# lenskit/csr

Measured on AMD Instinct MI355X. Metric: spmv_gflops, higher is better.
Workload: dtype f64

## Files before the change

### csr_amd/csrc/spmv.hip

```cpp
#include "spmv_plan.h"

#include <algorithm>
#include <ctime>

namespace csrk {
template <bool R32>
__device__ __forceinline__ double spmv_prod(double a, double x)
{
    const double t = a * x;
    return R32 ? (double)(float)t : t;
}

void free_spmv_plan(SpmvPlan *p) { delete p; }

void spmv_plan_bytes_by_part(const SpmvPlan *p, int64_t out[5])
{
    for (int i = 0; i < 5; i++) out[i] = 0;
    auto add = [&](int part, std::initializer_list<const DevBuf *> bufs) {
        for (const DevBuf *b : bufs) out[part] += (int64_t)b->bytes;
    };
    for (const AccPanel *ap : p->acc) add(0, {&ap->row_list, &ap->vals, &ap->idx, &ap->tile_row0, &ap->segs, &ap->wg_seg, &ap->partial, &ap->z});
    const Panel &t = p->tier1;
    add(1, {&t.row_list, &t.rp, &t.ci, &t.vs, &t.tile, &t.group, &t.carry_row, &t.carry_val, &t.y, &t.crp, &t.cidx});
    const LightStream *l = &p->ls;
    add(2, {&l->vals, &l->idx, &l->rowids, &l->tile_base, &l->carry_row, &l->carry_val});
    add(3, {&l->xg, &l->a_col, &l->a_dst, &l->blk_start, &l->round_start, &l->round_tile0, &l->wg_round0, &p->hot_slot, &p->hot_cols, &p->xh});
    add(4, {&p->tile_row, &p->carry_row, &p->carry_val, &p->rp_light, &p->cut_pos, &p->cut_cum, &p->tile_cut, &p->heavy_row, &p->seg_off,
            &p->seg_row, &p->seg_part, &p->xwide});
}

int64_t spmv_plan_bytes(const SpmvPlan *p)
{
    int64_t part[5];
    spmv_plan_bytes_by_part(p, part);
    return part[0] + part[1] + part[2] + part[3] + part[4];
}
// ... 217 lines not shown
            }
        }
    }
}

template <class XT>
__global__ void hot_pack_kernel(const XT *__restrict__ x, const int32_t *__restrict__ hot_cols, int32_t n_hot,
                                double *__restrict__ xh)
{
    const int i = blockIdx.x * blockDim.x + threadIdx.x;
    if (i < n_hot) xh[i] = (double)x[hot_cols[i]];
}

struct PanelRider {
    int64_t first;
    const double *partial;
    double *z;
    int32_t H, n_wg;
};

template <class PP, int PT, bool R32 = false, class XT = double>
__global__ __launch_bounds__(PT) void spmv_panel_kernel(
    const PP *__restrict__ prp, const int32_t *__restrict__ pci, const double *__restrict__ pvs,
    const XT *__restrict__ x, int32_t ncols, double *__restrict__ yp, const PanelTile *__restrict__ tiles,
    const PanelGroup *__restrict__ groups, int64_t n_prows, int32_t *__restrict__ carry_row,
    double *__restrict__ carry_val, int64_t pnnz, int32_t cb, PanelRider rider)
{
    constexpr uint32_t POS_MASK = (1u << PANEL_POS_BITS) - 1;
    __shared__ double s_buf[MERGE_ITEMS + 1];
    __shared__ int32_t s_long[MERGE_MAXLONG];
    __shared__ int32_t s_nlong;
    __shared__ double s_wpart[PT / WAVE];

    constexpr int PPAIRS = MERGE_ITEMS / PT / 2;
    const int tid = threadIdx.x;
    const int lane = tid & (WAVE - 1), wv = tid / WAVE;
    if ((int64_t)blockIdx.x >= rider.first) {
        constexpr int G = PT / WAVE;
        const int h = (int)((int64_t)blockIdx.x - rider.first) * WAVE + lane;
        const int per = (rider.n_wg + G - 1) / G;
        const int w0 = wv * per, w1 = w0 + per < rider.n_wg ? w0 + per : rider.n_wg;
        double acc = 0.0;
        if (h < rider.H) {
#pragma unroll 8
            for (int w = w0; w < w1; w++) acc += rider.partial[(int64_t)w * rider.H + h];
        }
        s_buf[wv * WAVE + lane] = acc;
        __syncthreads();
        if (wv == 0 && h < rider.H) {
            double tot = s_buf[lane];
            for (int u = 1; u < G; u++) tot += s_buf[u * WAVE + lane];
            rider.z[h] = tot;
        }
        return;
    }
    const PanelGroup grp = groups[blockIdx.x];
    if (grp.nt == 0) return;
    constexpr int RPT = MERGE_ITEMS / PT;
    int32_t c0[PPAIRS], c1[PPAIRS], rv[RPT];
    double p0[PPAIRS], p1[PPAIRS];
    PanelTile pt = tiles[grp.t0];

#define PANEL_LOAD_TILE(T)                                                                            \
    {                                                                                                 \
        const int64_t j0_ = (T).j0;                                                                   \
        const int nn_ = (T).nn, nr_ = (T).i1 - (T).i0;                                                \
        _Pragma("unroll") for (int u = 0; u < PPAIRS; u++)                                       \
// ... 92 lines not shown
            acc = wave_sum(acc);
            if (lane == 0) {
                if (r < nr) {
                    yp[i0 + r] = acc;
                } else {
                    *(pt.cslot >= 0 ? yp + pt.cslot : carry_val + t) = acc;
                }
            }
        }
        pt = nx;
    }
#undef PANEL_LOAD_TILE
}

template <int CB, int PT, bool R32 = false, class SV = double, class XT = double>
__global__ __launch_bounds__(PT) void spmv_acc_kernel(const SV *__restrict__ pvals, const uint16_t *__restrict__ pidx,
                                                     const int32_t *__restrict__ tile_row0,
                                                     const XT *__restrict__ x, int32_t ncols,
                                                     const AccSeg *__restrict__ segs, const int32_t *__restrict__ wg_seg,
                                                     int32_t H, double *__restrict__ partial, int32_t fx_g)
{
    extern __shared__ __align__(16) unsigned char acc_smem[];
    double *s_x = (double *)acc_smem;
    double *s_acc = s_x + CB + 2;
    const int Hpad = (H + 1) & ~1;
    double *s_hval = s_acc + Hpad;
    int32_t *s_hrow = (int32_t *)(s_hval + ACC_SEG_TILES);
    constexpr int NW = PT / WAVE;
    const int tid = threadIdx.x, lane = tid & (WAVE - 1), wv = tid / WAVE;

    for (int h = tid; h < Hpad; h += PT) s_acc[h] = 0.0;
    if (tid < 2) s_x[CB + tid] = 0.0;
    const unsigned long long below = lane ? (~0ull >> (WAVE - lane)) : 0ull;
    const unsigned long long upto = below | (1ull << lane);

    int cur_blk = -1;
    const int sb = wg_seg[blockIdx.x], se = wg_seg[blockIdx.x + 1];
    for (int si = sb; si < se; si++) {
        const AccSeg sg = segs[si];
        if (sg.blk != cur_blk) {
            cur_blk = sg.blk;
            const int32_t w0 = sg.blk * CB;
            const int wlen = ncols - w0 < CB ? ncols - w0 : CB;
            if (wlen == CB) {
                constexpr int WL = CB / 2 / PT;
                f64x2_t v[WL];
#pragma unroll
                for (int u = 0; u < WL; u++) {
                    if (sizeof(XT) == 8) {
                        v[u] = *((const F64x2 *)(x + w0) + tid + u * PT);
                    } else {
                        const f32x2_t t = *((const F32x2 *)(x + w0) + tid + u * PT);
// ... 2 lines not shown
                    }
                }
#pragma unroll
                for (int u = 0; u < WL; u++) ((f64x2_t *)s_x)[tid + u * PT] = v[u];
            } else {
                for (int k = tid; k < wlen; k += PT) s_x[k] = (double)x[w0 + k];
            }
        }
        __syncthreads();

        const int nt = sg.ntiles;
        AccVals<SV> v, vn;
        u32x4_t ix, ixn;
        int32_t tr0 = 0, tr0n = 0;
        int t = wv;
        const int64_t pstep = (int64_t)gridDim.x;
        if (t < nt) {
            const u32x4_t *ip = (const u32x4_t *)(pidx + (sg.ptile0 + t * pstep) * ACC_TILE);
            v.load(pvals + (sg.ptile0 + t * pstep) * ACC_TILE, lane);
            ix = __builtin_nontemporal_load(ip + lane);
            tr0 = tile_row0[sg.tile0 + t];
        }
        for (; t < nt; t += NW) {
            const bool more = t + NW < nt;
            if (more) {
                const u32x4_t *ip = (const u32x4_t *)(pidx + (sg.ptile0 + (t + NW) * pstep) * ACC_TILE);
                vn.load(pvals + (sg.ptile0 + (t + NW) * pstep) * ACC_TILE, lane);
                ixn = __builtin_nontemporal_load(ip + lane);
                tr0n = tile_row0[sg.tile0 + t + NW];
            }
            const uint32_t e[ACC_K] = {ix.x & 0xffffu, ix.x >> 16, ix.y & 0xffffu, ix.y >> 16,
// ... 73 lines not shown
        __syncthreads();
        if (wv == 0) {
            for (int base = 0; base < nt; base += WAVE) {
                const int i = base + lane;
                const bool ok = i < nt;
                const int row = ok ? s_hrow[i] : -1 - lane;
                const double val = ok ? s_hval[i] : 0.0;
                const int row_prev = wave_up1_i32(row, -2 - WAVE);
                const double S = wave_segscan(val, lane == 0 || row_prev != row, lane);
                const int row_next = wave_down1_i32(row, -2 - WAVE);
                if (ok && (lane == WAVE - 1 || row_next != row)) atomicAdd(&s_acc[row], S);
            }
        }
    }
    __syncthreads();
    for (int h = tid; h < H; h += PT) partial[(int64_t)blockIdx.x * H + h] = s_acc[h];
}

struct EpiJob {
    int32_t kind, blocks;
    const int32_t *carry_row;
    const double *carry_val;
    int64_t n;
    double *fy;
    const double *partial;
    const int32_t *row_list;
    int32_t H, n_wg, G;
    int32_t extra;
    const int32_t *crp, *cidx;
    const double *cval;
};
// ... 585 lines not shown
            const unsigned gs = (unsigned)(ceil_div(p->ls.n_stage_blk, 8) * 8);
            ls_stage_kernel<XT><<<gs, LS_STAGE_THREADS, (size_t)p->ls.stage_w * 8, s>>>(
                d_x, m->ncols, p->ls.stage_w, p->ls.a_col.as<uint16_t>(), p->ls.a_dst.as<int32_t>(),
                p->ls.blk_start.as<int32_t>(), p->ls.n_stage_blk, p->ls.xg.as<double>());
            ks.stop();
            CSRK_LAUNCH_CHECK();
        }
        if (do_light && p->n_hot && !(p->ls.on && p->ls.n_cold)) {
            hot_pack_kernel<XT><<<(unsigned)ceil_div(p->n_hot, 256), 256, 0, s>>>(d_x, p->hot_cols.as<int32_t>(), p->n_hot,
                                                                            p->xh.as<double>());
            CSRK_LAUNCH_CHECK();
        }
        bool t0_rides = false;
        if (do_heavy && p->n_heavy && !p->acc.empty()) {
            KernelTimer kh(p, s, 1);
            for (AccPanel *ap : p->acc) {
#define ACC_LAUNCH(SV)                                                                                                 \
    spmv_acc_kernel<ACC_CB, ACC_THREADS, R32, SV, XT><<<(unsigned)ap->n_wg, ACC_THREADS, ap->lds, s>>>(                \
        ap->vals.as<SV>(), ap->idx.as<uint16_t>(), ap->tile_row0.as<int32_t>(), d_x, m->ncols, ap->segs.as<AccSeg>(),  \
        ap->wg_seg.as<int32_t>(), ap->nrow, ap->partial.as<double>(), ap->fx_g)
                if (ap->f32) ACC_LAUNCH(float);
                else if (ap->fix56) ACC_LAUNCH(fix56::Packed);
                else ACC_LAUNCH(double);
#undef ACC_LAUNCH
                CSRK_LAUNCH_CHECK();
            }
            kh.stop();
        }
        if (do_heavy && p->n_heavy && p->tier1.on) {
            Panel *pn = &p->tier1;
            KernelTimer kh(p, s, 2);
#define PANEL_ARGS(PP)                                                                                              \
    pn->rp.as<PP>(), pn->ci.as<int32_t>(), pn->vs.as<double>(), d_x, m->ncols, pn->y.as<double>(),                    \
        pn->tile.as<PanelTile>(), pn->group.as<PanelGroup>(), pn->rows, pn->carry_row.as<int32_t>(),                  \
        pn->carry_val.as<double>(), pn->nnz, pn->cb, rider
            PanelRider rider = {pn->groups, nullptr, nullptr, 0, 0};
            if (PANEL_T1 / WAVE == 4 && do_heavy && p->acc.size() == 1 && p->acc[0]->z.p) {
                AccPanel *ap = p->acc[0];
                rider.partial = ap->partial.as<double>();
                rider.z = ap->z.as<double>();
                rider.H = ap->nrow;
                rider.n_wg = ap->n_wg;
                t0_rides = true;
            }
            const unsigned grid = (unsigned)(pn->groups + (t0_rides ? ceil_div(rider.H, WAVE) : 0));
            if (pn->p64) spmv_panel_kernel<int64_t, PANEL_T1, R32, XT><<<grid, PANEL_T1, 0, s>>>(PANEL_ARGS(int64_t));
            else spmv_panel_kernel<int32_t, PANEL_T1, R32, XT><<<grid, PANEL_T1, 0, s>>>(PANEL_ARGS(int32_t));
#undef PANEL_ARGS
            kh.stop();
            CSRK_LAUNCH_CHECK();
        }
        if (do_light) {
#define MERGE_ARGS_LIGHT(CI)                                                                                        \
    p->rp_light.as<P>(), CI, m->d_values, d_x, d_y, p->tile_row.as<int32_t>(), m->nrows, p->nnz_light,                \
        p->carry_row.as<int32_t>(), p->carry_val.as<double>(), p->tile_cut.as<int32_t>(), p->cut_pos.as<int64_t>(),  \
        p->cut_cum.as<int64_t>(), m->nnz
#define MERGE_ARGS_FULL(CI)                                                                                         \
    rp, CI, m->d_values, d_x, d_y, p->tile_row.as<int32_t>(), m->nrows, m->nnz, p->carry_row.as<int32_t>(),          \
        p->carry_val.as<double>(), nullptr, nullptr, nullptr, m->nnz
            const unsigned grid = (unsigned)p->n_tiles;
// ... 53 lines not shown
            if (p->n_heavy)
                spmv_merge_fixup_short_kernel<<<(unsigned)ceil_div(p->n_tiles, 256), 256, 0, s>>>(
                    p->carry_row.as<int32_t>(), p->carry_val.as<double>(), p->n_tiles, d_y);
            else
                spmv_merge_fixup_kernel<<<(unsigned)ceil_div(p->n_tiles * WAVE, 256), 256, 0, s>>>(
                    p->carry_row.as<int32_t>(), p->carry_val.as<double>(), p->n_tiles, d_y);
            CSRK_LAUNCH_CHECK();
            } else {
                set_error("internal: a float32 vector reached the raw-array kernels");
                return CSRK_ERR_INVALID;
            }
#undef MERGE_ARGS_LIGHT
#undef MERGE_ARGS_FULL
        }
        if (do_heavy && p->n_heavy && !p->acc.empty() && t0_rides) {
            AccPanel *ap = p->acc[0];
            if (epi.n == 6) CSRK_TRY(flush_epi());
            EpiJob J = {};
            J.kind = 2;
            J.blocks = (int32_t)ceil_div(ap->nrow, EPI_THREADS);
            J.partial = ap->z.as<double>();
            J.row_list = ap->row_list.as<int32_t>();
            J.H = ap->nrow;
            epi.j[epi.n++] = J;
        } else if (do_heavy && p->n_heavy && !p->acc.empty())
            for (AccPanel *ap : p->acc)
                CSRK_TRY(add_red(ap->partial.as<double>(), ap->row_list.as<int32_t>(), ap->nrow, ap->n_wg, 4, nullptr, nullptr, nullptr));
        if (do_heavy && p->n_heavy && p->tier1.on) {
            Panel *pn = &p->tier1;
            CSRK_TRY(add_red(pn->y.as<double>(), pn->row_list.as<int32_t>(), pn->nrow, pn->nb, pn->nb > 64 ? 4 : 2,
                             pn->crp.as<int32_t>(), pn->cidx.as<int32_t>(), pn->carry_val.as<double>(), pn->ncs));
        }
        CSRK_TRY(flush_epi());
        break;
    }
    case CSRK_SPMV_VECTOR: {
        if constexpr (!X64) {
            set_error("internal: a float32 vector reached the raw-array kernels");
            return CSRK_ERR_INVALID;
// ... 309 lines not shown
    float ms4[4] = {0.f, 0.f, 0.f, 0.f};
    CSRK_REQUIRE(n_records && mean_ms, "output is NULL");
    CSRK_TRY(csrk_spmv_profile_end4(h, n_records, ms4));
    for (int c = 0; c < 3; c++) mean_ms[c] = ms4[c];
    return CSRK_OK;
}

int csrk_spmv_plan_stats(csrk_handle_t h, int64_t *out, int n)
{
    Matrix *m = from_handle(h);
    if (!m) return CSRK_ERR_INVALID;
    CSRK_REQUIRE(out && n >= 0, "out is NULL");
    SpmvPlan *p = nullptr;
    CSRK_TRY(get_plan(m, nullptr, &p));
    const Panel &t1 = p->tier1;
    int64_t a_tiles = 0, a_rows = 0, a_nnz = 0, a_nb = 0;
    for (const AccPanel *ap : p->acc) {
        a_tiles += ap->tiles;
        a_rows += ap->nrow;
        a_nnz += ap->nnz;
        a_nb = ap->nb;
    }
    const bool af = !p->acc.empty();
    const int64_t plan_bytes = spmv_plan_bytes(p);
    int64_t part[5];
    spmv_plan_bytes_by_part(p, part);
    const int64_t v[34] = {p->algo == CSRK_SPMV_MERGE ? p->n_tiles : p->n_segs,
                           p->algo == CSRK_SPMV_MERGE ? p->tile_items : VEC_SEG,
                           p->n_heavy, p->algo == CSRK_SPMV_MERGE ? p->nnz_light : m->nnz,
                           a_tiles, a_nb, p->heavy_min, af ? ACC_CB : 0, p->n_heavy ? 2 : 0, a_rows, a_nnz,
                           t1.nrow, t1.rows, t1.nnz, p->tier1_min, t1.cb,
                           p->n_hot, (int64_t)(p->hot_cover * 1e6), af ? 1 : 0, p->hot_slots,
                           p->ls.on ? 1 : 0, p->ls.n_tiles, p->ls.n_runs, p->ls.grid, p->ls.n_cold, plan_bytes,
                           p->ls.round_start.p ? p->ls.stage_tiles : 0,
                           af ? (int64_t)p->acc[0]->n_wg : 0, 0, part[0], part[1], part[2], part[3], part[4]};
    for (int i = 0; i < n && i < 34; i++) out[i] = v[i];
    const LightStream &ls = p->ls;
    const bool rnd = ls.on && ls.n_cold && ls.round_start.p;
    const int64_t plain_rounds = ls.on ? ceil_div(ls.n_tiles, LS_THREADS / WAVE) : 0;
    const int64_t w[8] = {ls.on && ls.dense ? 1 : 0,
                          ls.on && ls.idx24 ? 1 : 0,
                          ls.on ? p->n_hot_lds : 0,
                          rnd ? ls.n_rounds : plain_rounds,
                          rnd ? ls.max_wg_rounds : (ls.on ? ceil_div(plain_rounds, (int64_t)ls.grid) : 0),
                          rnd ? ls.n_stage_blk : 0,
                          rnd ? ls.stage_w : 0,
                          ls.on && ls.f32 ? 1 : 0};
    for (int i = 34; i < n && i < 42; i++) out[i] = w[i - 34];
    return CSRK_OK;
}
// ... 24 lines not shown
```

### csr_amd/csrc/spmv_plan.h

```cpp
#pragma once
#include "common.h"
#include "wave.h"
#include "fix56.h"

#include <vector>

namespace csrk {

template <int VT> struct ValLoad;
template <> struct ValLoad<CSRK_VAL_F64> {
    static __device__ __forceinline__ double at(const void *v, int64_t k) { return ((const double *)v)[k]; }
};
template <> struct ValLoad<CSRK_VAL_F32> {
    static __device__ __forceinline__ double at(const void *v, int64_t k) { return (double)((const float *)v)[k]; }
};
template <> struct ValLoad<CSRK_VAL_NONE> {
    static __device__ __forceinline__ double at(const void *, int64_t) { return 1.0; }
};

__device__ __forceinline__ double wave_sum(double v)
{
#pragma unroll
    for (int off = WAVE / 2; off > 0; off >>= 1) v += __shfl_down(v, off, WAVE);
    return v;
// ... 21 lines not shown
    DevBuf row_list;
    DevBuf rp, ci, vs, tile, group, carry_row, carry_val, y;
    int32_t ncs = 0;
    DevBuf crp, cidx;
};

struct AccSeg {
    int64_t tile0;
    int64_t ptile0;
    int32_t ntiles;
    int32_t blk;
};

struct AccPanel {
    int32_t nrow = 0, nb = 0, n_wg = 0;
    int64_t tiles = 0, nnz = 0, n_segs = 0;
    size_t lds = 0;
    DevBuf row_list, vals, idx, tile_row0, segs, wg_seg, partial;
    DevBuf z;
    bool f32 = false;
    bool fix56 = false;
    int32_t fx_g = 0;
};

struct LightStream {
    bool on = false;
    int64_t n_tiles = 0;
    int32_t n_runs = 0, n_out = 0;
    unsigned grid = 0;
    DevBuf vals, idx, rowids, tile_base, carry_row, carry_val;
// ... 25 lines not shown
    DevBuf cut_cum;
    DevBuf tile_cut;
    DevBuf heavy_row;
    int32_t n_hot = 0;
    int32_t n_hot_lds = 0;
    int32_t hot_slots = 0;
    double hot_cover = 0.0;
    DevBuf hot_slot;
    DevBuf hot_cols;
    DevBuf xh;
    Panel tier1;
    LightStream ls;
    std::vector<int32_t> t1_rows;
    int64_t t1_nnz = 0;
    std::vector<AccPanel *> acc;
    std::vector<int32_t> t0_rows;
    std::vector<int64_t> t0_lens;
    int64_t n_segs = 0;
    DevBuf seg_off;
    DevBuf seg_row;
    DevBuf seg_part;
    DevBuf xwide;
    std::vector<hipEvent_t> ev;
    std::vector<int> ev_chan;
    int ev_used = 0;
    bool profiling = false;
    int prof_every = 1;
    int prof_calls = 0;
    int prof_mask = 0xf;
    bool prof_this = false;
// ... 58 lines not shown
    int32_t nn;
    int32_t blk;
};
constexpr int PANEL_CARRY_ROWS = 4;

struct PanelGroup {
    int64_t t0;
    int32_t nt;
    int32_t blk;
};
constexpr int ACC_CB = 4096;
constexpr int ACC_K = 8;
constexpr int ACC_TILE = WAVE * ACC_K;
constexpr int ACC_MAXROWS = 15936;
constexpr int ACC_FLOOR = 128;
constexpr int ACC_SEG_TILES = 256;
constexpr int ACC_THREADS = 1024;
constexpr int ACC_ROW_SHIFT = 13;
constexpr uint32_t ACC_COL_MASK = (1u << ACC_ROW_SHIFT) - 1;
constexpr int ACC_MAXSTEP = 7;

typedef uint32_t u32x4_t __attribute__((ext_vector_type(4)));
typedef uint32_t u32x2_t __attribute__((ext_vector_type(2)));

__host__ __device__ __forceinline__ int acc_val_slot(int e)
{
    const int lane = e >> 3, j = e & 7;
    return (j >> 1) * (2 * WAVE) + lane * 2 + (j & 1);
}
__host__ __device__ __forceinline__ int acc_idx_slot(int e)
{
    const int lane = e >> 3, j = e & 7;
    return (j >> 2) * (4 * WAVE) + lane * 4 + (j & 3);
}
template <class SV> __host__ __device__ __forceinline__ int acc_slot_of(int e)
// ... 115 lines not shown
```

### csr_amd/csrc/spmv_plan.hip

```cpp
#include "spmv_plan.h"

#include <algorithm>
#include <cstring>
#include <ctime>
#include <type_traits>

namespace csrk {
struct PlanTrace {
    bool on;
    double t0;
    static double now()
    {
        timespec ts;
        clock_gettime(CLOCK_MONOTONIC, &ts);
        return ts.tv_sec * 1e3 + ts.tv_nsec * 1e-6;
    }
    PlanTrace() : on(getenv("CSRK_PLAN_TRACE") != nullptr), t0(0.0)
    {
        if (on) {
            (void)hipDeviceSynchronize();
            t0 = now();
        }
    }
    void lap(const char *what)
// ... 877 lines not shown
    pn->ncs = ncs;
    CSRK_HIP(hipStreamSynchronize(s));
    tr.lap("  tier 1: groups, carries (host)");
    pn->on = true;
    pn->cb = cb;
    pn->nb = nb;
    pn->nrow = n;
    pn->rows = pairs;
    pn->tiles = n_tiles;
    pn->nnz = nnz_rows;
    return CSRK_OK;
}

template <class P, int VT>
static int build_acc_panel(Matrix *m, AccPanel *ap, const int32_t *rows, const int64_t *lens, int32_t n, int64_t nnz_rows,
                           hipStream_t s)
{
    const P *rp = (const P *)m->d_rowptrs;
    const int32_t nb = (int32_t)ceil_div(m->ncols > 0 ? m->ncols : 1, ACC_CB);
    PlanTrace tr;
    const int64_t pairs = (int64_t)n * nb;
    CSRK_TRY(ap->row_list.alloc((size_t)n * 4));
    CSRK_TRY(stage_h2d(ap->row_list.p, rows, (size_t)n * 4, s));
    DevBuf off, bends, pstart, d_trow, d_tpiece;
    CSRK_TRY(off.alloc((size_t)(pairs + 1) * 8));
    std::vector<int32_t> trow, tpiece;
    for (int32_t c = 0; c < n; c++)
        for (int64_t pc = 0; pc * ACC_PIECE < lens[c]; pc++) {
            trow.push_back(c);
            tpiece.push_back((int32_t)pc);
        }
    const int64_t n_tasks = (int64_t)trow.size();
// ... 15 lines not shown
    CSRK_LAUNCH_CHECK();
    CSRK_TRY(exclusive_scan_i64(off.as<int64_t>(), off.as<int64_t>(), pairs, s));
    CSRK_TRY(bends.alloc((size_t)(nb + 1) * 8));
    panel_blockends_kernel<<<(unsigned)ceil_div(nb + 1, 256), 256, 0, s>>>(off.as<int64_t>(), n, nb, bends.as<int64_t>());
    CSRK_LAUNCH_CHECK();
    std::vector<int64_t> be((size_t)nb + 1), t0((size_t)nb + 1);
    CSRK_TRY(stage_d2h(be.data(), bends.p, (size_t)(nb + 1) * 8, s));
    CSRK_HIP(hipStreamSynchronize(s));
    t0[0] = 0;
    for (int32_t b = 0; b < nb; b++) t0[b + 1] = t0[b] + ceil_div(be[b + 1] - be[b], ACC_TILE);
    const int64_t n_tiles = t0[nb];
    CSRK_TRY(stage_h2d(bends.p, t0.data(), (size_t)(nb + 1) * 8, s));
    tr.lap("  tier 0: counts, gaps, scan");
    int cus = 0;
    CSRK_HIP(hipDeviceGetAttribute(&cus, hipDeviceAttributeMultiprocessorCount, m->device));
    int64_t n_wg = cus > 0 ? cus : 256;
    if (n_wg > n_tiles) n_wg = n_tiles;
    if (n_wg < 1) n_wg = 1;
    std::vector<int64_t> wg_t0((size_t)n_wg + 1);
    int64_t share_max = 0;
    for (int64_t w = 0; w <= n_wg; w++) wg_t0[(size_t)w] = n_tiles * w / n_wg;
    for (int64_t w = 0; w < n_wg; w++) share_max = std::max(share_max, wg_t0[(size_t)w + 1] - wg_t0[(size_t)w]);
    const int64_t n_phys = share_max * n_wg;
    DevBuf d_wg_t0;
    CSRK_TRY(d_wg_t0.alloc((size_t)(n_wg + 1) * 8));
    CSRK_TRY(stage_h2d(d_wg_t0.p, wg_t0.data(), (size_t)(n_wg + 1) * 8, s));
    ap->f32 = VT == CSRK_VAL_F32;
    DevBuf fx;
    CSRK_TRY(fx.alloc(16));
    if (VT == CSRK_VAL_F64 && n > 0) {
        const char *env = getenv("CSRK_SPMV_FIX56");
        if (!(env && env[0] == '0')) {
            int32_t h[4] = {0, INT32_MAX, INT32_MIN, 0};
            CSRK_TRY(stage_h2d(fx.p, h, sizeof h, s));
            acc_range_kernel<P><<<dim3((unsigned)n, 16), 256, 0, s>>>(rp, (const double *)m->d_values, ap->row_list.as<int32_t>(),
                                                                     fx.as<int32_t>());
            CSRK_LAUNCH_CHECK();
            CSRK_TRY(stage_d2h(h, fx.p, sizeof h, s));
            CSRK_HIP(hipStreamSynchronize(s));
            fix56::Range r;
            r.bad = h[0];
            r.lo = h[1];
            r.hi = h[2];
            ap->fix56 = fix56::packable(r, ap->fx_g);
            tr.lap("  tier 0: value grid test");
// ... 61 lines not shown
    CSRK_TRY(ap->segs.alloc(segs.size() * sizeof(AccSeg)));
    CSRK_TRY(ap->wg_seg.alloc(wg_seg.size() * 4));
    CSRK_TRY(stage_h2d(ap->segs.p, segs.data(), segs.size() * sizeof(AccSeg), s));
    CSRK_TRY(stage_h2d(ap->wg_seg.p, wg_seg.data(), wg_seg.size() * 4, s));
    CSRK_TRY(ap->partial.alloc((size_t)n_wg * n * 8));
    CSRK_TRY(ap->z.alloc((size_t)n * 8));
    ap->lds = (size_t)(ACC_CB + 2) * 8 + (size_t)((n + 1) & ~1) * 8 + (size_t)ACC_SEG_TILES * 12;
    CSRK_TRY(spmv_kernel_attributes());
    CSRK_HIP(hipStreamSynchronize(s));
    ap->nrow = n;
    ap->nb = nb;
    ap->n_wg = (int32_t)n_wg;
    ap->tiles = n_tiles;
    ap->nnz = nnz_rows;
    ap->n_segs = (int64_t)segs.size();
    tr.lap("  tier 0: segments");
    return CSRK_OK;
}


template <class P>
static int build_heavy_split(Matrix *m, SpmvPlan *p, hipStream_t s, bool allow_tier1 = true)
{
    p->n_heavy = 0;
    const char *env = getenv("CSRK_SPMV_HEAVY_SPLIT");
    if (env && env[0] == '0') return CSRK_OK;
    HEAVY_MIN = 2048;
    TIERB_MIN = TIERB_MIN_DEFAULT;
    if (const char *e = getenv("CSRK_HEAVY_MIN")) HEAVY_MIN = atoi(e) > 64 ? atoi(e) : 64;
    if (const char *e = getenv("CSRK_TIERB_MIN")) TIERB_MIN = atoi(e) >= 0 ? atoi(e) : 0;
    const bool tier1 = allow_tier1 && TIERB_MIN > 0 && TIERB_MIN < HEAVY_MIN;
    const int cut_min = tier1 ? TIERB_MIN : HEAVY_MIN;
// ... 32 lines not shown
    heavy_sorted_kernel<P><<<(unsigned)n_cut, 1024, 0, s>>>(rp, m->d_colinds, p->heavy_row.as<int32_t>(), n_cut,
                                                         bad.as<int32_t>());
    CSRK_LAUNCH_CHECK();
    tr.lap("  split: view + sorted kernels");
    int32_t is_bad = 0;
    std::vector<int32_t> rows((size_t)n_cut);
    std::vector<int64_t> lens((size_t)n_cut);
    CSRK_TRY(stage_d2h(&is_bad, bad.p, 4, s));
    CSRK_TRY(stage_d2h(rows.data(), p->heavy_row.p, (size_t)n_cut * 4, s));
    CSRK_TRY(stage_d2h(lens.data(), clen.p, (size_t)n_cut * 8, s));
    CSRK_HIP(hipStreamSynchronize(s));
    if (tr.on) fprintf(stderr, "[csrk plan]   n_cut %d\n", n_cut);
    tr.lap("  split: copies to the host");
    if (is_bad) return CSRK_OK;

    if (tier1 && !getenv("CSRK_HEAVY_MIN")) {
        int64_t n_min = 0;
        for (int32_t c = 0; c < n_cut; c++) n_min += lens[c] >= HEAVY_MIN;
        if (n_min < ACC_MAXROWS && n_cut > n_min) {
            const size_t kth = (size_t)(n_cut < ACC_MAXROWS ? n_cut : ACC_MAXROWS) - 1;
            int64_t thr = -1;
            {
                constexpr int64_t HB = 1 << 16;
                std::vector<int32_t> hist((size_t)HB + 1, 0);
                for (int32_t c = 0; c < n_cut; c++) hist[(size_t)(lens[c] < HB ? lens[c] : HB)]++;
                int64_t seen = hist[(size_t)HB];
                if (seen <= (int64_t)kth)
                    for (int64_t v = HB - 1; v >= 0; v--) {
                        seen += hist[(size_t)v];
                        if (seen > (int64_t)kth) {
                            thr = v;
                            break;
                        }
                    }
            }
            if (thr < 0) {
                std::vector<int64_t> sl(lens);
                std::nth_element(sl.begin(), sl.begin() + kth, sl.end(), [](int64_t a, int64_t b) { return a > b; });
                thr = sl[kth];
            }
            int64_t n_ge = 0;
            for (int32_t c = 0; c < n_cut; c++) n_ge += lens[c] >= thr;
            if (n_ge > ACC_MAXROWS) thr++;
            thr = thr < ACC_FLOOR ? ACC_FLOOR : thr;
            if (thr < HEAVY_MIN) HEAVY_MIN = (int)thr;
        }
    }
    p->heavy_min = HEAVY_MIN;
    p->tier1_min = TIERB_MIN;
    std::vector<int32_t> r0, r1;
    std::vector<int64_t> len0;
    int64_t nnz1 = 0;
    r0.reserve((size_t)n_cut);
    r1.reserve((size_t)n_cut);
    len0.reserve((size_t)n_cut);
    for (int32_t c = 0; c < n_cut; c++) {
        if (lens[c] >= HEAVY_MIN) {
            r0.push_back(rows[c]);
// ... 5 lines not shown
    }
    const int64_t pair_cap = 256ll << 20;
    const int64_t pairs1 = (int64_t)r1.size() * ceil_div(m->ncols > 0 ? m->ncols : 1, PANEL_CB1);
    if (pairs1 > pair_cap && tier1) return build_heavy_split<P>(m, p, s, false);

    p->n_heavy = n_cut;
    p->nnz_light = m->nnz - nnz_cut;
    p->t0_rows = std::move(r0);
    p->t0_lens = std::move(len0);
    p->t1_rows = std::move(r1);
    p->t1_nnz = nnz1;
    tr.lap("  split: host lists");
    return CSRK_OK;
}

template <class P>
static int build_tiers(Matrix *m, SpmvPlan *p, hipStream_t s)
{
    if (!p->n_heavy) return CSRK_OK;
    const std::vector<int32_t> &r0 = p->t0_rows, &r1 = p->t1_rows;
    const std::vector<int64_t> &len0 = p->t0_lens;
    const int64_t nnz1 = p->t1_nnz;
#define BUILD(VT)                                                                                                  \
    do {                                                                                                           \
        for (size_t g0 = 0; g0 < r0.size(); g0 += ACC_MAXROWS) {                                                   \
            const size_t g1 = g0 + ACC_MAXROWS < r0.size() ? g0 + ACC_MAXROWS : r0.size();                         \
            int64_t gn = 0;                                                                                        \
            for (size_t c = g0; c < g1; c++) gn += len0[c];                                                        \
            AccPanel *ap = new (std::nothrow) AccPanel();                                                          \
            CSRK_REQUIRE(ap, "out of host memory");                                                                \
            p->acc.push_back(ap);                                                                                  \
            CSRK_TRY((build_acc_panel<P, VT>(m, ap, r0.data() + g0, len0.data() + g0, (int32_t)(g1 - g0), gn, s)));  \
        }                                                                                                          \
        if (!r1.empty()) CSRK_TRY((build_panel<P, VT>(m, &p->tier1, r1, nnz1, PANEL_CB1, 1, true, s)));            \
    } while (0)
    if (m->val_type == CSRK_VAL_F64) BUILD(CSRK_VAL_F64);
    else if (m->val_type == CSRK_VAL_F32) BUILD(CSRK_VAL_F32);
    else BUILD(CSRK_VAL_NONE);
#undef BUILD
    return CSRK_OK;
}

template <class P>
static int build_hot_cache(Matrix *m, SpmvPlan *p, hipStream_t s)
{
    p->n_hot = 0;
    const char *env = getenv("CSRK_SPMV_HOT");
    if (env && env[0] == '0') return CSRK_OK;
// ... 629 lines not shown
```

Measured before the change: 799.6.

## Split heavy-row tier into concurrent row groups sharing one launch with XCD placement

Heavy rows (tier 0) can now be dealt round-robin by length into up to three groups. Each group gets its own accumulation panel and a share of the CUs, and all groups run in a single acc-kernel launch through a workgroup map that spreads groups across the 8 XCDs. The threshold for heavy rows widens to group count times the row cap, so more rows go to the accumulator path instead of tier 1. The panel kernel's rider reduction and the epilogue now handle multiple groups. A group-count heuristic decides whether to split, and fix56 compression is turned off for a group's panels whenever any panel in that group is stored raw. The risk is extra per-group overhead and more partial-reduction traffic.

After: 827.4, median of 6. +3.5%, better.

```diff
diff --git a/csr_amd/csrc/acc_groups.h b/csr_amd/csrc/acc_groups.h
--- /dev/null
+++ b/csr_amd/csrc/acc_groups.h
@@ -0,0 +1,111 @@
+#pragma once
+#include <algorithm>
+#include <cstdint>
+#include <numeric>
+#include <vector>
+
+namespace csrk {
+namespace accgroups {
+
+constexpr int MAX_GROUPS = 3;
+constexpr int XCDS = 8;
+
+struct Deal {
+    std::vector<std::vector<int32_t>> groups;
+    std::vector<int32_t> first;
+};
+
+inline Deal deal_rows(const int64_t *lens, int32_t n, int G, int32_t cap)
+{
+    Deal d;
+    d.first.push_back(0);
+    if (n <= 0) return d;
+    if (cap < 1) cap = 1;
+    if (G < 1) G = 1;
+    if (G > MAX_GROUPS) G = MAX_GROUPS;
+    if (G == 1) {
+        for (int32_t g0 = 0; g0 < n; g0 += cap) {
+            const int32_t g1 = n - g0 < cap ? n : g0 + cap;
+            std::vector<int32_t> g((size_t)(g1 - g0));
+            std::iota(g.begin(), g.end(), g0);
+            d.groups.push_back(std::move(g));
+            d.first.push_back((int32_t)d.groups.size());
+        }
+        return d;
+    }
+    std::vector<int32_t> rank((size_t)n);
+    std::iota(rank.begin(), rank.end(), 0);
+    std::stable_sort(rank.begin(), rank.end(), [&](int32_t a, int32_t b) { return lens[a] > lens[b]; });
+    const int64_t per_launch = (int64_t)G * cap;
+    for (int64_t r0 = 0; r0 < n; r0 += per_launch) {
+        const int64_t nl = n - r0 < per_launch ? n - r0 : per_launch;
+        const int gb = (int)std::min<int64_t>(G, (nl + cap - 1) / cap);
+        const size_t base = d.groups.size();
+        d.groups.resize(base + (size_t)gb);
+        for (int64_t i = 0; i < nl; i++) d.groups[base + (size_t)(i % gb)].push_back(rank[(size_t)(r0 + i)]);
+        for (int g = 0; g < gb; g++) std::sort(d.groups[base + (size_t)g].begin(), d.groups[base + (size_t)g].end());
+        d.first.push_back((int32_t)d.groups.size());
+    }
+    return d;
+}
+
+constexpr int64_t TILE_ENTRIES = 512;
+constexpr int64_t MIN_SEG_TILES = 48;
+inline int choose_groups(const int64_t *lens, int32_t n, int g_max, int32_t cap, int64_t floor_len, int64_t nb, int32_t cus)
+{
+    if (cap < 1) cap = 1;
+    if (g_max > MAX_GROUPS) g_max = MAX_GROUPS;
+    if (g_max < 2 || n <= cap) return 1;
+    std::vector<int64_t> sl;
+    for (int32_t i = 0; i < n; i++)
+        if (lens[i] >= floor_len) sl.push_back(lens[i]);
+    for (int g = g_max; g > 1; g--) {
+        const int64_t k = std::min<int64_t>((int64_t)sl.size(), (int64_t)g * cap);
+        if (k <= (int64_t)(g - 1) * cap) continue;
+        if (k < (int64_t)sl.size()) std::nth_element(sl.begin(), sl.begin() + k, sl.end(), [](int64_t a, int64_t b) { return a > b; });
+        int64_t entries = 0;
+        for (int64_t i = 0; i < k; i++) entries += sl[(size_t)i];
+        if (entries / TILE_ENTRIES >= MIN_SEG_TILES * ((int64_t)g * nb + cus)) return g;
+    }
+    return 1;
+}
+
+inline int32_t group_wgs(int32_t cus, int gb, int g)
+{
+    const int32_t n = cus / gb + (g < cus % gb ? 1 : 0);
+    return n < 1 ? 1 : n;
+}
+
+inline std::vector<uint32_t> place_wgs(const int32_t *n_wg, int gb)
+{
+    int64_t total = 0;
+    int32_t w_max = 0;
+    for (int g = 0; g < gb; g++) {
+        total += n_wg[g];
+        w_max = std::max(w_max, n_wg[g]);
+    }
+    std::vector<uint32_t> map((size_t)total, ~0u);
+    int64_t fill[XCDS], room[XCDS];
+    for (int c = 0; c < XCDS; c++) {
+        fill[c] = 0;
+        room[c] = total / XCDS + (c < total % XCDS ? 1 : 0);
+    }
+    std::vector<uint32_t> late;
+    for (int32_t w = 0; w < w_max; w++)
+        for (int g = 0; g < gb; g++) {
+            if (w >= n_wg[g]) continue;
+            const uint32_t id = ((uint32_t)g << 16) | (uint32_t)w;
+            const int c = w % XCDS;
+            if (fill[c] < room[c]) map[(size_t)(c + XCDS * fill[c]++)] = id;
+            else late.push_back(id);
+        }
+    size_t b = 0;
+    for (uint32_t id : late) {
+        while (map[b] != ~0u) b++;
+        map[b] = id;
+    }
+    return map;
+}
+
+}
+}
diff --git a/csr_amd/csrc/spmv.hip b/csr_amd/csrc/spmv.hip
--- a/csr_amd/csrc/spmv.hip
+++ b/csr_amd/csrc/spmv.hip
@@ -19,7 +19,7 @@
     auto add = [&](int part, std::initializer_list<const DevBuf *> bufs) {
         for (const DevBuf *b : bufs) out[part] += (int64_t)b->bytes;
     };
-    for (const AccPanel *ap : p->acc) add(0, {&ap->row_list, &ap->vals, &ap->idx, &ap->tile_row0, &ap->segs, &ap->wg_seg, &ap->partial, &ap->z});
+    for (const AccPanel *ap : p->acc) add(0, {&ap->row_list, &ap->vals, &ap->idx, &ap->tile_row0, &ap->segs, &ap->wg_seg, &ap->partial, &ap->z, &ap->wg_map});
     const Panel &t = p->tier1;
     add(1, {&t.row_list, &t.rp, &t.ci, &t.vs, &t.tile, &t.group, &t.carry_row, &t.carry_val, &t.y, &t.crp, &t.cidx});
     const LightStream *l = &p->ls;
@@ -267,9 +267,9 @@
 
 struct PanelRider {
     int64_t first;
-    const double *partial;
-    double *z;
-    int32_t H, n_wg;
+    const double *partial[accgroups::MAX_GROUPS];
+    double *z[accgroups::MAX_GROUPS];
+    int32_t H[accgroups::MAX_GROUPS], n_wg[accgroups::MAX_GROUPS], start[accgroups::MAX_GROUPS];
 };
 
 template <class PP, int PT, bool R32 = false, class XT = double>
@@ -290,20 +290,34 @@
     const int lane = tid & (WAVE - 1), wv = tid / WAVE;
     if ((int64_t)blockIdx.x >= rider.first) {
         constexpr int G = PT / WAVE;
-        const int h = (int)((int64_t)blockIdx.x - rider.first) * WAVE + lane;
-        const int per = (rider.n_wg + G - 1) / G;
-        const int w0 = wv * per, w1 = w0 + per < rider.n_wg ? w0 + per : rider.n_wg;
+        int rb = (int)((int64_t)blockIdx.x - rider.first);
+        const double *__restrict__ partial = rider.partial[0];
+        double *__restrict__ z = rider.z[0];
+        int32_t H = rider.H[0], n_wg = rider.n_wg[0], start = 0;
+#pragma unroll
+        for (int q = 1; q < accgroups::MAX_GROUPS; q++)
+            if (rb >= rider.start[q]) {
+                partial = rider.partial[q];
+                z = rider.z[q];
+                H = rider.H[q];
+                n_wg = rider.n_wg[q];
+                start = rider.start[q];
+            }
+        rb -= start;
+        const int h = rb * WAVE + lane;
+        const int per = (n_wg + G - 1) / G;
+        const int w0 = wv * per, w1 = w0 + per < n_wg ? w0 + per : n_wg;
         double acc = 0.0;
-        if (h < rider.H) {
+        if (h < H) {
 #pragma unroll 8
-            for (int w = w0; w < w1; w++) acc += rider.partial[(int64_t)w * rider.H + h];
+            for (int w = w0; w < w1; w++) acc += partial[(int64_t)w * H + h];
         }
         s_buf[wv * WAVE + lane] = acc;
         __syncthreads();
-        if (wv == 0 && h < rider.H) {
+        if (wv == 0 && h < H) {
             double tot = s_buf[lane];
             for (int u = 1; u < G; u++) tot += s_buf[u * WAVE + lane];
-            rider.z[h] = tot;
+            z[h] = tot;
         }
         return;
     }
@@ -426,12 +440,23 @@
 }
 
 template <int CB, int PT, bool R32 = false, class SV = double, class XT = double>
-__global__ __launch_bounds__(PT) void spmv_acc_kernel(const SV *__restrict__ pvals, const uint16_t *__restrict__ pidx,
-                                                     const int32_t *__restrict__ tile_row0,
-                                                     const XT *__restrict__ x, int32_t ncols,
-                                                     const AccSeg *__restrict__ segs, const int32_t *__restrict__ wg_seg,
-                                                     int32_t H, double *__restrict__ partial, int32_t fx_g)
-{
+__global__ __launch_bounds__(PT) void spmv_acc_kernel(const AccLaunchArgs L, const XT *__restrict__ x, int32_t ncols)
+{
+    uint32_t grp = 0, wg = blockIdx.x;
+    if (L.wg_map) {
+        const uint32_t id = L.wg_map[blockIdx.x];
+        grp = id >> 16;
+        wg = id & 0xffffu;
+    }
+    const AccGroupArgs &A = L.g[grp];
+    const SV *__restrict__ pvals = (const SV *)A.vals;
+    const uint16_t *__restrict__ pidx = A.idx;
+    const int32_t *__restrict__ tile_row0 = A.tile_row0;
+    const AccSeg *__restrict__ segs = A.segs;
+    const int32_t *__restrict__ wg_seg = A.wg_seg;
+    double *__restrict__ partial = A.partial;
+    const int32_t H = A.H;
+    const int32_t fx_g = A.fx_g;
     extern __shared__ __align__(16) unsigned char acc_smem[];
     double *s_x = (double *)acc_smem;
     double *s_acc = s_x + CB + 2;
@@ -447,7 +472,7 @@
     const unsigned long long upto = below | (1ull << lane);
 
     int cur_blk = -1;
-    const int sb = wg_seg[blockIdx.x], se = wg_seg[blockIdx.x + 1];
+    const int sb = wg_seg[wg], se = wg_seg[wg + 1];
     for (int si = sb; si < se; si++) {
         const AccSeg sg = segs[si];
         if (sg.blk != cur_blk) {
@@ -480,7 +505,7 @@
         u32x4_t ix, ixn;
         int32_t tr0 = 0, tr0n = 0;
         int t = wv;
-        const int64_t pstep = (int64_t)gridDim.x;
+        const int64_t pstep = (int64_t)A.n_wg;
         if (t < nt) {
             const u32x4_t *ip = (const u32x4_t *)(pidx + (sg.ptile0 + t * pstep) * ACC_TILE);
             v.load(pvals + (sg.ptile0 + t * pstep) * ACC_TILE, lane);
@@ -584,7 +609,7 @@
         }
     }
     __syncthreads();
-    for (int h = tid; h < H; h += PT) partial[(int64_t)blockIdx.x * H + h] = s_acc[h];
+    for (int h = tid; h < H; h += PT) partial[(int64_t)wg * H + h] = s_acc[h];
 }
 
 struct EpiJob {
@@ -1200,11 +1225,24 @@
         bool t0_rides = false;
         if (do_heavy && p->n_heavy && !p->acc.empty()) {
             KernelTimer kh(p, s, 1);
-            for (AccPanel *ap : p->acc) {
-#define ACC_LAUNCH(SV)                                                                                                 \
-    spmv_acc_kernel<ACC_CB, ACC_THREADS, R32, SV, XT><<<(unsigned)ap->n_wg, ACC_THREADS, ap->lds, s>>>(                \
-        ap->vals.as<SV>(), ap->idx.as<uint16_t>(), ap->tile_row0.as<int32_t>(), d_x, m->ncols, ap->segs.as<AccSeg>(),  \
-        ap->wg_seg.as<int32_t>(), ap->nrow, ap->partial.as<double>(), ap->fx_g)
+            for (size_t a0 = 0; a0 < p->acc.size(); a0 += (size_t)p->acc[a0]->launch_groups) {
+                AccPanel *ap = p->acc[a0];
+                const int gb = ap->launch_groups;
+                if (gb < 1 || gb > accgroups::MAX_GROUPS || a0 + (size_t)gb > p->acc.size()) {
+                    set_error("internal: tier 0's groups and launches disagree");
+                    return CSRK_ERR_INVALID;
+                }
+                AccLaunchArgs L = {};
+                size_t lds = 0;
+                for (int g = 0; g < gb; g++) {
+                    const AccPanel *aq = p->acc[a0 + (size_t)g];
+                    L.g[g] = {aq->vals.p, aq->idx.as<uint16_t>(), aq->tile_row0.as<int32_t>(), aq->segs.as<AccSeg>(),
+                              aq->wg_seg.as<int32_t>(), aq->partial.as<double>(), aq->nrow, aq->n_wg, aq->fx_g, 0};
+                    lds = aq->lds > lds ? aq->lds : lds;
+                }
+                L.wg_map = gb > 1 ? ap->wg_map.as<uint32_t>() : nullptr;
+                const unsigned n_blocks = (unsigned)(gb > 1 ? ap->launch_wgs : ap->n_wg);
+#define ACC_LAUNCH(SV) spmv_acc_kernel<ACC_CB, ACC_THREADS, R32, SV, XT><<<n_blocks, ACC_THREADS, lds, s>>>(L, d_x, m->ncols)
                 if (ap->f32) ACC_LAUNCH(float);
                 else if (ap->fix56) ACC_LAUNCH(fix56::Packed);
                 else ACC_LAUNCH(double);
@@ -1220,16 +1258,24 @@
     pn->rp.as<PP>(), pn->ci.as<int32_t>(), pn->vs.as<double>(), d_x, m->ncols, pn->y.as<double>(),                    \
         pn->tile.as<PanelTile>(), pn->group.as<PanelGroup>(), pn->rows, pn->carry_row.as<int32_t>(),                  \
         pn->carry_val.as<double>(), pn->nnz, pn->cb, rider
-            PanelRider rider = {pn->groups, nullptr, nullptr, 0, 0};
-            if (PANEL_T1 / WAVE == 4 && do_heavy && p->acc.size() == 1 && p->acc[0]->z.p) {
-                AccPanel *ap = p->acc[0];
-                rider.partial = ap->partial.as<double>();
-                rider.z = ap->z.as<double>();
-                rider.H = ap->nrow;
-                rider.n_wg = ap->n_wg;
+            PanelRider rider = {};
+            rider.first = pn->groups;
+            for (int q = 0; q < accgroups::MAX_GROUPS; q++) rider.start[q] = INT32_MAX;
+            int64_t rider_wgs = 0;
+            if (PANEL_T1 / WAVE == 4 && do_heavy && !p->acc.empty() && (size_t)p->acc[0]->launch_groups == p->acc.size() &&
+                p->acc.size() <= (size_t)accgroups::MAX_GROUPS && p->acc[0]->z.p) {
+                for (size_t q = 0; q < p->acc.size(); q++) {
+                    AccPanel *ap = p->acc[q];
+                    rider.partial[q] = ap->partial.as<double>();
+                    rider.z[q] = ap->z.as<double>();
+                    rider.H[q] = ap->nrow;
+                    rider.n_wg[q] = ap->n_wg;
+                    rider.start[q] = (int32_t)rider_wgs;
+                    rider_wgs += ceil_div(ap->nrow, WAVE);
+                }
                 t0_rides = true;
             }
-            const unsigned grid = (unsigned)(pn->groups + (t0_rides ? ceil_div(rider.H, WAVE) : 0));
+            const unsigned grid = (unsigned)(pn->groups + rider_wgs);
             if (pn->p64) spmv_panel_kernel<int64_t, PANEL_T1, R32, XT><<<grid, PANEL_T1, 0, s>>>(PANEL_ARGS(int64_t));
             else spmv_panel_kernel<int32_t, PANEL_T1, R32, XT><<<grid, PANEL_T1, 0, s>>>(PANEL_ARGS(int32_t));
 #undef PANEL_ARGS
@@ -1313,15 +1359,16 @@
 #undef MERGE_ARGS_FULL
         }
         if (do_heavy && p->n_heavy && !p->acc.empty() && t0_rides) {
-            AccPanel *ap = p->acc[0];
-            if (epi.n == 6) CSRK_TRY(flush_epi());
-            EpiJob J = {};
-            J.kind = 2;
-            J.blocks = (int32_t)ceil_div(ap->nrow, EPI_THREADS);
-            J.partial = ap->z.as<double>();
-            J.row_list = ap->row_list.as<int32_t>();
-            J.H = ap->nrow;
-            epi.j[epi.n++] = J;
+            for (AccPanel *ap : p->acc) {
+                if (epi.n == 6) CSRK_TRY(flush_epi());
+                EpiJob J = {};
+                J.kind = 2;
+                J.blocks = (int32_t)ceil_div(ap->nrow, EPI_THREADS);
+                J.partial = ap->z.as<double>();
+                J.row_list = ap->row_list.as<int32_t>();
+                J.H = ap->nrow;
+                epi.j[epi.n++] = J;
+            }
         } else if (do_heavy && p->n_heavy && !p->acc.empty())
             for (AccPanel *ap : p->acc)
                 CSRK_TRY(add_red(ap->partial.as<double>(), ap->row_list.as<int32_t>(), ap->nrow, ap->n_wg, 4, nullptr, nullptr, nullptr));
@@ -1661,8 +1708,9 @@
     SpmvPlan *p = nullptr;
     CSRK_TRY(get_plan(m, nullptr, &p));
     const Panel &t1 = p->tier1;
-    int64_t a_tiles = 0, a_rows = 0, a_nnz = 0, a_nb = 0;
+    int64_t a_tiles = 0, a_rows = 0, a_nnz = 0, a_nb = 0, a_wgs = 0;
     for (const AccPanel *ap : p->acc) {
+        a_wgs += ap->n_wg;
         a_tiles += ap->tiles;
         a_rows += ap->nrow;
         a_nnz += ap->nnz;
@@ -1680,7 +1728,7 @@
                            p->n_hot, (int64_t)(p->hot_cover * 1e6), af ? 1 : 0, p->hot_slots,
                            p->ls.on ? 1 : 0, p->ls.n_tiles, p->ls.n_runs, p->ls.grid, p->ls.n_cold, plan_bytes,
                            p->ls.round_start.p ? p->ls.stage_tiles : 0,
-                           af ? (int64_t)p->acc[0]->n_wg : 0, 0, part[0], part[1], part[2], part[3], part[4]};
+                           a_wgs, 0, part[0], part[1], part[2], part[3], part[4]};
     for (int i = 0; i < n && i < 34; i++) out[i] = v[i];
     const LightStream &ls = p->ls;
     const bool rnd = ls.on && ls.n_cold && ls.round_start.p;
diff --git a/csr_amd/csrc/spmv_plan.h b/csr_amd/csrc/spmv_plan.h
--- a/csr_amd/csrc/spmv_plan.h
+++ b/csr_amd/csrc/spmv_plan.h
@@ -2,6 +2,7 @@
 #include "common.h"
 #include "wave.h"
 #include "fix56.h"
+#include "acc_groups.h"
 
 #include <vector>
 
@@ -59,6 +60,8 @@
 
 struct AccPanel {
     int32_t nrow = 0, nb = 0, n_wg = 0;
+    int32_t launch_groups = 1, launch_wgs = 0;
+    DevBuf wg_map;
     int64_t tiles = 0, nnz = 0, n_segs = 0;
     size_t lds = 0;
     DevBuf row_list, vals, idx, tile_row0, segs, wg_seg, partial;
@@ -114,6 +117,7 @@
     std::vector<int32_t> t1_rows;
     int64_t t1_nnz = 0;
     std::vector<AccPanel *> acc;
+    int acc_groups = 1;
     std::vector<int32_t> t0_rows;
     std::vector<int64_t> t0_lens;
     int64_t n_segs = 0;
@@ -202,11 +206,27 @@
 constexpr int ACC_TILE = WAVE * ACC_K;
 constexpr int ACC_MAXROWS = 15936;
 constexpr int ACC_FLOOR = 128;
+constexpr int ACC_GROUPS_DEFAULT = 2;
+static_assert(accgroups::TILE_ENTRIES == ACC_TILE, "acc_groups.h counts the streams' tiles");
 constexpr int ACC_SEG_TILES = 256;
 constexpr int ACC_THREADS = 1024;
 constexpr int ACC_ROW_SHIFT = 13;
 constexpr uint32_t ACC_COL_MASK = (1u << ACC_ROW_SHIFT) - 1;
 constexpr int ACC_MAXSTEP = 7;
+
+struct AccGroupArgs {
+    const void *vals;
+    const uint16_t *idx;
+    const int32_t *tile_row0;
+    const AccSeg *segs;
+    const int32_t *wg_seg;
+    double *partial;
+    int32_t H, n_wg, fx_g, pad_;
+};
+struct AccLaunchArgs {
+    AccGroupArgs g[accgroups::MAX_GROUPS];
+    const uint32_t *wg_map;
+};
 
 typedef uint32_t u32x4_t __attribute__((ext_vector_type(4)));
 typedef uint32_t u32x2_t __attribute__((ext_vector_type(2)));
diff --git a/csr_amd/csrc/spmv_plan.hip b/csr_amd/csrc/spmv_plan.hip
--- a/csr_amd/csrc/spmv_plan.hip
+++ b/csr_amd/csrc/spmv_plan.hip
@@ -915,8 +915,10 @@
 
 template <class P, int VT>
 static int build_acc_panel(Matrix *m, AccPanel *ap, const int32_t *rows, const int64_t *lens, int32_t n, int64_t nnz_rows,
-                           hipStream_t s)
-{
+                           hipStream_t s, int32_t wg_want = 0, bool allow_fix56 = true)
+{
+    ap->fix56 = false;
+    ap->fx_g = 0;
     const P *rp = (const P *)m->d_rowptrs;
     const int32_t nb = (int32_t)ceil_div(m->ncols > 0 ? m->ncols : 1, ACC_CB);
     PlanTrace tr;
@@ -962,7 +964,7 @@
     tr.lap("  tier 0: counts, gaps, scan");
     int cus = 0;
     CSRK_HIP(hipDeviceGetAttribute(&cus, hipDeviceAttributeMultiprocessorCount, m->device));
-    int64_t n_wg = cus > 0 ? cus : 256;
+    int64_t n_wg = wg_want > 0 ? wg_want : cus > 0 ? cus : 256;
     if (n_wg > n_tiles) n_wg = n_tiles;
     if (n_wg < 1) n_wg = 1;
     std::vector<int64_t> wg_t0((size_t)n_wg + 1);
@@ -976,7 +978,7 @@
     ap->f32 = VT == CSRK_VAL_F32;
     DevBuf fx;
     CSRK_TRY(fx.alloc(16));
-    if (VT == CSRK_VAL_F64 && n > 0) {
+    if (VT == CSRK_VAL_F64 && n > 0 && allow_fix56) {
         const char *env = getenv("CSRK_SPMV_FIX56");
         if (!(env && env[0] == '0')) {
             int32_t h[4] = {0, INT32_MAX, INT32_MIN, 0};
@@ -1068,8 +1070,25 @@
     ap->tiles = n_tiles;
     ap->nnz = nnz_rows;
     ap->n_segs = (int64_t)segs.size();
+    if (tr.on)
+        fprintf(stderr, "[csrk plan]   tier 0 group: rows %d entries %lld workgroups %lld tiles %lld, %.1f per segment%s\n", n,
+                (long long)nnz_rows, (long long)n_wg, (long long)n_tiles, segs.empty() ? 0.0 : (double)n_tiles / (double)segs.size(),
+                ap->fix56 ? " (fix56)" : "");
     tr.lap("  tier 0: segments");
     return CSRK_OK;
+}
+
+static int acc_groups_knob()
+{
+    const char *e = getenv("CSRK_ACC_GROUPS");
+    const int g = e ? atoi(e) : ACC_GROUPS_DEFAULT;
+    return g < 1 ? 1 : g > accgroups::MAX_GROUPS ? accgroups::MAX_GROUPS : g;
+}
+static int32_t acc_group_rows_knob()
+{
+    const char *e = getenv("CSRK_ACC_GROUP_ROWS");
+    const int r = e ? atoi(e) : ACC_MAXROWS;
+    return r < 1 || r > ACC_MAXROWS ? ACC_MAXROWS : r;
 }
 
 
@@ -1132,11 +1151,21 @@
     tr.lap("  split: copies to the host");
     if (is_bad) return CSRK_OK;
 
+    p->acc_groups = acc_groups_knob();
+    if (!getenv("CSRK_ACC_GROUPS")) {
+        int cus = 0;
+        CSRK_HIP(hipDeviceGetAttribute(&cus, hipDeviceAttributeMultiprocessorCount, m->device));
+        const bool extend = tier1 && !getenv("CSRK_HEAVY_MIN");
+        p->acc_groups = accgroups::choose_groups(lens.data(), n_cut, ACC_GROUPS_DEFAULT, acc_group_rows_knob(),
+                                                 extend ? (int64_t)std::max(ACC_FLOOR, cut_min) : (int64_t)HEAVY_MIN,
+                                                 ceil_div(m->ncols > 0 ? m->ncols : 1, ACC_CB), cus > 0 ? cus : 256);
+    }
+    const int64_t t0_cap = (int64_t)p->acc_groups * acc_group_rows_knob();
     if (tier1 && !getenv("CSRK_HEAVY_MIN")) {
         int64_t n_min = 0;
         for (int32_t c = 0; c < n_cut; c++) n_min += lens[c] >= HEAVY_MIN;
-        if (n_min < ACC_MAXROWS && n_cut > n_min) {
-            const size_t kth = (size_t)(n_cut < ACC_MAXROWS ? n_cut : ACC_MAXROWS) - 1;
+        if (n_min < t0_cap && n_cut > n_min) {
+            const size_t kth = (size_t)(n_cut < t0_cap ? n_cut : t0_cap) - 1;
             int64_t thr = -1;
             {
                 constexpr int64_t HB = 1 << 16;
@@ -1159,7 +1188,7 @@
             }
             int64_t n_ge = 0;
             for (int32_t c = 0; c < n_cut; c++) n_ge += lens[c] >= thr;
-            if (n_ge > ACC_MAXROWS) thr++;
+            if (n_ge > t0_cap) thr++;
             thr = thr < ACC_FLOOR ? ACC_FLOOR : thr;
             if (thr < HEAVY_MIN) HEAVY_MIN = (int)thr;
         }
@@ -1195,24 +1224,70 @@
     return CSRK_OK;
 }
 
+template <class P, int VT>
+static int build_acc_groups(Matrix *m, SpmvPlan *p, hipStream_t s)
+{
+    const std::vector<int32_t> &r0 = p->t0_rows;
+    const std::vector<int64_t> &len0 = p->t0_lens;
+    if (r0.empty()) return CSRK_OK;
+    const accgroups::Deal deal = accgroups::deal_rows(len0.data(), (int32_t)r0.size(), p->acc_groups, acc_group_rows_knob());
+    int cus = 0;
+    CSRK_HIP(hipDeviceGetAttribute(&cus, hipDeviceAttributeMultiprocessorCount, m->device));
+    if (cus <= 0) cus = 256;
+    std::vector<int32_t> rows;
+    std::vector<int64_t> lens;
+    for (size_t j = 0; j + 1 < deal.first.size(); j++) {
+        const int k0 = deal.first[j], gb = deal.first[j + 1] - k0;
+        const size_t a0 = p->acc.size();
+        auto build = [&](int g, bool allow_fix56) -> int {
+            const std::vector<int32_t> &pos = deal.groups[(size_t)(k0 + g)];
+            rows.resize(pos.size());
+            lens.resize(pos.size());
+            int64_t gn = 0;
+            for (size_t i = 0; i < pos.size(); i++) {
+                rows[i] = r0[(size_t)pos[i]];
+                lens[i] = len0[(size_t)pos[i]];
+                gn += lens[i];
+            }
+            return build_acc_panel<P, VT>(m, p->acc[a0 + (size_t)g], rows.data(), lens.data(), (int32_t)pos.size(), gn, s,
+                                          gb > 1 ? accgroups::group_wgs(cus, gb, g) : 0, allow_fix56);
+        };
+        bool any_raw = false;
+        for (int g = 0; g < gb; g++) {
+            AccPanel *ap = new (std::nothrow) AccPanel();
+            CSRK_REQUIRE(ap, "out of host memory");
+            p->acc.push_back(ap);
+            CSRK_TRY(build(g, true));
+            any_raw = any_raw || !ap->fix56;
+        }
+        AccPanel *head = p->acc[a0];
+        if (gb == 1) continue;
+        for (int g = 0; g < gb; g++)
+            if (any_raw && p->acc[a0 + (size_t)g]->fix56) CSRK_TRY(build(g, false));
+        int32_t n_wg[accgroups::MAX_GROUPS];
+        for (int g = 0; g < gb; g++) {
+            n_wg[g] = p->acc[a0 + (size_t)g]->n_wg;
+            p->acc[a0 + (size_t)g]->launch_groups = 0;
+        }
+        const std::vector<uint32_t> map = accgroups::place_wgs(n_wg, gb);
+        head->launch_groups = gb;
+        head->launch_wgs = (int32_t)map.size();
+        CSRK_TRY(head->wg_map.alloc(map.size() * 4));
+        CSRK_TRY(stage_h2d(head->wg_map.p, map.data(), map.size() * 4, s));
+        CSRK_HIP(hipStreamSynchronize(s));
+    }
+    return CSRK_OK;
+}
+
 template <class P>
 static int build_tiers(Matrix *m, SpmvPlan *p, hipStream_t s)
 {
     if (!p->n_heavy) return CSRK_OK;
-    const std::vector<int32_t> &r0 = p->t0_rows, &r1 = p->t1_rows;
-    const std::vector<int64_t> &len0 = p->t0_lens;
+    const std::vector<int32_t> &r1 = p->t1_rows;
     const int64_t nnz1 = p->t1_nnz;
 #define BUILD(VT)                                                                                                  \
     do {                                                                                                           \
-        for (size_t g0 = 0; g0 < r0.size(); g0 += ACC_MAXROWS) {                                                   \
-            const size_t g1 = g0 + ACC_MAXROWS < r0.size() ? g0 + ACC_MAXROWS : r0.size();                         \
-            int64_t gn = 0;                                                                                        \
-            for (size_t c = g0; c < g1; c++) gn += len0[c];                                                        \
-            AccPanel *ap = new (std::nothrow) AccPanel();                                                          \
-            CSRK_REQUIRE(ap, "out of host memory");                                                                \
-            p->acc.push_back(ap);                                                                                  \
-            CSRK_TRY((build_acc_panel<P, VT>(m, ap, r0.data() + g0, len0.data() + g0, (int32_t)(g1 - g0), gn, s)));  \
-        }                                                                                                          \
+        CSRK_TRY((build_acc_groups<P, VT>(m, p, s)));                                                              \
         if (!r1.empty()) CSRK_TRY((build_panel<P, VT>(m, &p->tier1, r1, nnz1, PANEL_CB1, 1, true, s)));            \
     } while (0)
     if (m->val_type == CSRK_VAL_F64) BUILD(CSRK_VAL_F64);
```
